# zubair-irshad/NeO-360

Hardware: AMD Instinct MI355X
Metric: rays/sec (128 samples/ray) + PSNR vs ref, 640x480 (higher is better)
Workload: dtype f32 (fp16-MFMA products of hi/lo-split fp32 operands, fp32 accumulate)

## Files before the change

neo-360_amd/csrc/api_tp.hip:

```cpp
#include "tp_frame.h"

#include <algorithm>

using namespace neo_host;

namespace {

double tp_flop_per_point(int input_ch, int nv) {
    const double per_view = input_ch == 3 ? 255424.0 : 260800.0;
    return 2.0 * (nv * per_view + 4416.0);
}

int ensure_projections(neo_ctx* ctx, MlpSlot& sl, const neo::TpScene& sc, bool planes, hipStream_t s, long plane_base[3],
                       bool split_guard = false) {
    const long t_lat = static_cast<long>(sc.nv) * sc.Hf * sc.Wf, t_pl = static_cast<long>(sc.nv) * sc.Hp * sc.Wp;
    for (int j = 0; j < 3; ++j) plane_base[j] = t_lat + j * t_pl;
    const size_t need = neo::tp_proj_bytes(t_lat + (planes ? 3 * t_pl : 0)) + neo::tp_proj_pad_bytes();
    REQUIRE(need <= 4294967295UL, "projected maps too large for 32-bit byte offsets");
    if (need > sl.proj.cap) {
        if (int rc = ctx->touch_shared(s)) return rc;
        if (sl.proj.reserve(need)) return NEO_ERR_NOMEM;
        sl.proj_weights = sl.proj_scene = sl.projpl_weights = sl.projpl_scene = 0;
    }
    if (sl.proj_weights != sl.weights_epoch || sl.proj_scene != ctx->scene_epoch) {
        if (int rc = ctx->touch_shared(s)) return rc;
        neo::launch_tp_preproject(sc.latent, t_lat, sl.wpack.as<float>(), neo::tp_kc_x(sl.input_ch), sl.proj.as<float>(), s);
        if (split_guard) neo::launch_f32_range_check(sl.proj.as<float>(), static_cast<size_t>(t_lat) * 256, 65504.0f, ctx->flags, s);
        sl.proj_weights = sl.weights_epoch;
        sl.proj_scene = ctx->scene_epoch;
    }
    if (planes && (sl.projpl_weights != sl.weights_epoch || sl.projpl_scene != ctx->scene_epoch)) {
        if (int rc = ctx->touch_shared(s)) return rc;
        for (int j = 0; j < 3; ++j)
            neo::launch_tp_preproject(sc.plane[j], t_pl, sl.wpack.as<float>(), neo::tp_kc_x(sl.input_ch),
                                      sl.proj.as<float>() + plane_base[j] * 256, s, 256, 128, 64);
        if (split_guard)
            neo::launch_f32_range_check(sl.proj.as<float>() + plane_base[0] * 256, static_cast<size_t>(3 * t_pl) * 256, 65504.0f / 3.0f, ctx->flags, s);
        sl.projpl_weights = sl.weights_epoch;
        sl.projpl_scene = ctx->scene_epoch;
    }
    return NEO_OK;
}

int guard_planes_low(neo_ctx* ctx, const neo::TpScene& sc, hipStream_t s) {
    if (ctx->planes_low_checked == ctx->scene_epoch) return NEO_OK;
    if (int rc = ctx->touch_shared(s)) return rc;
    if (int rc = guard_map_low(ctx, MAP_MAX_PLANES, sc.plane, 3, static_cast<size_t>(sc.nv) * sc.Hp * sc.Wp * 128, neo::SPLIT_MAP_LOW,
                               true, s)) return rc;
    ctx->planes_low_checked = ctx->scene_epoch;
    return NEO_OK;
}

int tp_launch(neo_ctx* ctx, MlpSlot& sl, const neo::TpScene& sc, const neo::TpViews& views, const float* rays_o,
              const float* rays_d, const float* viewdirs, const float* tvals, const float* far, int R, int N, int chunk,
              float* out, hipStream_t s, const int* cull_map = nullptr, const int* cull_count = nullptr,
              bool density_only = false) {
    ORDERED(ctx, s);
    const int slot_index = static_cast<int>(&sl - ctx->tp);
    neo::TpScene scp = sc;
    if (cull_map) {
        scp.cull_map = cull_map;
        scp.cull_count = cull_count;
        scp.grid_w = 0;
    }
    if (scp.grid_w > 0) {
        static int epw = -2, eph = -2;
        if (epw == -2) {
            epw = eph = -1;
            if (const char* e = getenv("NEO_TP_PATCH")) (void)sscanf(e, "%d,%d", &epw, &eph);
        }
        scp.grid_pw = epw >= 0 ? epw : (slot_index < 2 ? 1 : 3);
        scp.grid_ph = eph >= 0 ? eph : (slot_index < 2 ? 1 : 3);
        if (scp.grid_w % (1 << scp.grid_pw) != 0) scp.grid_w = 0;
    }
    {
        static const int quad_default[4] = {16, 16, 16, 16};
        static int equad = -2;
        if (equad == -2) {
            const char* e = getenv("NEO_TP_QUAD");
            const int v = e ? atoi(e) : -1;
            equad = v == 1 ? 4 : (v == 0 || v == 4 || v == 8 || v == 16) ? v : -1;
        }
        const int forced = ctx->tp_quad >= 0 ? ctx->tp_quad : equad;
        scp.quad = cull_map ? 0 : forced >= 0 ? forced : quad_default[slot_index];
    }
    long plane_base[3] = {0, 0, 0};
    if (ctx->precision == 1) {
        if (ctx->planes_checked != ctx->scene_epoch) {
            const size_t n = static_cast<size_t>(sc.nv) * sc.Hp * sc.Wp * 128;
            for (int j = 0; j < 3; ++j) neo::launch_f32_range_check(sc.plane[j], n, 65504.0f / 3.0f, ctx->flags, s);
            ctx->planes_checked = ctx->scene_epoch;
        }
        if (ctx->preproject) {
            const bool planes = ctx->preproject == 2 || (ctx->preproject == 3 && slot_index >= 2);
            if (int rc = ensure_projections(ctx, sl, sc, planes, s, plane_base, true)) return rc;
            guard_split_weights(sl, sl.wpack_hp.p, neo::tp_wpack_hp_bytes(sl.input_ch), ctx->flags, s, neo::SPLIT_WEIGHT_LOW_TP, 1u << 6);
            if (!planes)
                if (int rc = guard_planes_low(ctx, sc, s)) return rc;
            neo::TpMlpHDev mh{sl.wpack_hp.p, sl.bias_hp.as<float>(), sl.heads.as<float>(), ctx->flags};
            const bool dens = density_only && !(cull_map && sl.input_ch == 3);
            if (ctx->tp_dirsum->reserve(static_cast<size_t>(R) * 32 * sizeof(float))) return NEO_ERR_NOMEM;
            if (!dens) neo::launch_tp_dirsum(viewdirs, R, views, sc.nv, ctx->tp_dirsum->as<float>(), s);
            ctx->span_kernel_next = planes ? 2 : 1;
            ctx->span_begin(s);
            if (planes)
                neo::launch_tp_mlp_hpp(sl.input_ch, mh, sl.proj.as<float>(), plane_base, scp, views, rays_o, rays_d, viewdirs, tvals, far,
                                       R, N, chunk, ctx->flags, out, ctx->tp_dirsum->as<float>(), s, dens);
            else
                neo::launch_tp_mlp_hp(sl.input_ch, mh, sl.proj.as<float>(), scp, views, rays_o, rays_d, viewdirs, tvals, far, R, N,
                                      chunk, ctx->flags, out, ctx->tp_dirsum->as<float>(), s, dens);
        } else {
            guard_split_weights(sl, sl.wpack_h.p, neo::tp_wpack_h_bytes(sl.input_ch), ctx->flags, s, neo::SPLIT_WEIGHT_LOW_TP);
            if (ctx->latent_checked != ctx->scene_epoch) {
                neo::launch_f32_range_check(sc.latent, static_cast<size_t>(sc.nv) * sc.Hf * sc.Wf * 512, 65504.0f, ctx->flags, s);
                ctx->latent_checked = ctx->scene_epoch;
            }
            if (int rc = guard_planes_low(ctx, sc, s)) return rc;
            if (ctx->latent_low_checked != ctx->scene_epoch) {
                if (int rc = ctx->touch_shared(s)) return rc;
                if (int rc = guard_map_low(ctx, MAP_MAX_LATENT, &sc.latent, 1, static_cast<size_t>(sc.nv) * sc.Hf * sc.Wf * 512,
                                           neo::SPLIT_MAP_LOW, true, s)) return rc;
                ctx->latent_low_checked = ctx->scene_epoch;
            }
            neo::TpMlpHDev mh{sl.wpack_h.p, sl.bias.as<float>(), sl.heads.as<float>(), ctx->flags};
            ctx->span_kernel_next = 3;
            ctx->span_begin(s);
            neo::launch_tp_mlp_h(sl.input_ch, mh, scp, views, rays_o, rays_d, viewdirs, tvals, far, R, N, chunk, ctx->flags, out, s);
        }
    } else {
        neo::TpMlpDev m{sl.wpack.as<float>(), sl.bias.as<float>(), sl.heads.as<float>()};
        const bool planes = ctx->preproject >= 2;
        if (ctx->preproject)
            if (int rc = ensure_projections(ctx, sl, sc, planes, s, plane_base)) return rc;
        const float* pbase = sl.proj.as<float>();
        const neo::TpPlaneProj pp{{pbase + plane_base[0] * 256, pbase + plane_base[1] * 256, pbase + plane_base[2] * 256}};
        if (ctx->preproject) {
            if (ctx->tp_dirsum->reserve(static_cast<size_t>(R) * 32 * sizeof(float))) return NEO_ERR_NOMEM;
            neo::launch_tp_dirsum(viewdirs, R, views, sc.nv, ctx->tp_dirsum->as<float>(), s);
        }
        ctx->span_kernel_next = 4;
        ctx->span_begin(s);
        neo::launch_tp_mlp(sl.input_ch, m, scp, views, rays_o, rays_d, viewdirs, tvals, far, R, N, chunk, ctx->flags, out, s,
                           ctx->preproject ? sl.proj.as<float>() : nullptr, planes ? &pp : nullptr,
                           ctx->preproject ? ctx->tp_dirsum->as<float>() : nullptr);
    }
    ctx->span_end(s, cull_map ? 0.0 : static_cast<double>(R) * N, tp_flop_per_point(sl.input_ch, sc.nv));
    return NEO_OK;
}

constexpr int SKIP_WINDOW_DEFAULT = 4096;

int tp_eval_skipping(neo_ctx* ctx, const TpFrame& f, const TpFrameArgs& a, int level, const float* fg_t, int N, float* fg_out,
                     uint8_t* keep, long long* kept) {
    hipStream_t s = f.s;
    const int win = std::min(ctx->skip_window > 0 ? ctx->skip_window : SKIP_WINDOW_DEFAULT, a.R);
    const size_t cap = static_cast<size_t>(win) * N;
    REQUIRE(cap * 3 <= 2147483647UL, "skip window too large for 32-bit indices");
    if (ctx->ws[12].reserve(neo::occ_rows_bytes(cap)) || (!keep && ctx->ws[13].reserve(cap))) return NEO_ERR_NOMEM;
    neo::OccRows w;
    w.carve(ctx->ws[12].p, cap);
    const uint32_t* bits = ctx->occ_G ? ctx->occ_bits.as<uint32_t>() : nullptr;
    if (kept) HIP_TRY(hipMemsetAsync(kept, 0, sizeof(long long), s));
    neo::launch_occ_iota(w.iota, static_cast<int>(cap), s);
    for (int r0 = 0; r0 < a.R; r0 += win) {
        const int rays = std::min(win, a.R - r0);
        const int P = rays * N;
        const size_t first = static_cast<size_t>(r0) * N;
        uint8_t* keep_win = keep ? keep + first : ctx->ws[13].as<uint8_t>();
        neo::launch_occ_compact(a.rays_o, a.rays_d, a.viewdirs, fg_t + first, r0, rays, a.R, N, a.chunk, bits, ctx->occ_G, keep_win,
                                w, kept, s);
        if (int rc = tp_launch(ctx, ctx->tp[level], f.sc, f.views, w.o, w.d, w.v, w.t, nullptr, P, 1, a.chunk, w.out, s, w.iota, w.count))
            return rc;
        neo::launch_occ_scatter(keep_win, P, w, fg_out + first * 4, s);
    }
    return NEO_OK;
}

struct TpTermState {
    double* carry;
    float* trans;
    int* stop;
    int* cws;
    static size_t bytes(size_t r, int win) { return r * 16 + neo::cull_ws_ints(win) * sizeof(int); }
    void carve(void* base, size_t r) {
        carry = static_cast<double*>(base);
        trans = reinterpret_cast<float*>(carry + r);
        stop = reinterpret_cast<int*>(trans + r);
        cws = stop + r;
    }
};

int tp_eval_terminating(neo_ctx* ctx, const TpFrame& f, const TpFrameArgs& a, int level, const float* fg_t, const float* far, int N,
                        float* fg_out, float eps, int segment, const TpTermState& st, int win, long long* kept) {
    hipStream_t s = f.s;
    const int seg = std::min(segment, N);
    const size_t cap = static_cast<size_t>(win) * seg;
    if (ctx->ws[12].reserve(neo::occ_rows_bytes(cap))) return NEO_ERR_NOMEM;
    neo::OccRows w;
    w.carve(ctx->ws[12].p, cap);
    HIP_TRY(hipMemsetAsync(fg_out, 0, static_cast<size_t>(a.R) * N * 16, s));
    neo::launch_term_init(st.trans, st.stop, a.R, 0, kept, 0, s);
    neo::launch_occ_iota(w.iota, static_cast<int>(cap), s);
    for (int r0 = 0; r0 < a.R; r0 += win) {
        const int rays = std::min(win, a.R - r0);
        for (int b0 = 0; b0 < N; b0 += segment) {
            const int len = std::min(segment, N - b0);
            const int P = rays * len;
            neo::launch_cull_compact(st.trans + r0, st.trans + r0, rays, eps, st.cws, nullptr, s);
            const int* map_w = neo::cull_map_of(st.cws, rays);
            const int* count_w = neo::cull_count_of(st.cws, rays);
            neo::launch_term_emit(a.rays_o, a.rays_d, a.viewdirs, fg_t, map_w, count_w, r0, rays, a.R, N, b0, len, a.chunk, w, kept, s);
            if (int rc = tp_launch(ctx, ctx->tp[level], f.sc, f.views, w.o, w.d, w.v, w.t, nullptr, P, 1, a.chunk, w.out, s, w.iota, w.count))
                return rc;
            neo::launch_term_scatter(w, P, fg_out, s);
            neo::launch_term_advance(fg_out, fg_t, a.rays_d, far, N, b0, b0 + len, segment, eps, map_w, count_w, rays, r0, st.carry,
                                     st.trans, st.stop, s);
        }
    }
    return NEO_OK;
}

bool level0_sigma_only(const neo_tp_level_out* level0) {
    return !level0 || !(level0->rgb || level0->fg_rgb || level0->bg_rgb || level0->depth);
}

}

int neo_tp_eval_region(neo_ctx* ctx, int slot, const neo::TpScene& sc, const neo::TpViews& views, const float* rays_o,
                       const float* rays_d, const float* viewdirs, const float* tvals, const float* far, int R, int N,
                       int chunk, float* out, hipStream_t s) {
    MlpSlot& sl = ctx->tp[slot];
    if (!sl.ready) return fail(NEO_ERR_STATE, "NeRF_TP MLP slot %d has no weights", slot);
    return tp_launch(ctx, sl, sc, views, rays_o, rays_d, viewdirs, tvals, far, R, N, chunk, out, s);
}

namespace neo_host {

int TpFrame::begin(neo_ctx* c, const TpFrameArgs& a, bool outside, bool use_grid, const Own& own) {
    ctx = c;
    s = static_cast<hipStream_t>(a.stream);
    REQUIRE(a.R >= 0 && a.chunk >= 1, "bad ray count / chunk");
    REQUIRE(!own.after_rays, own.after_rays);
    REQUIRE(a.n_coarse >= 3 && a.n_coarse <= 256 && a.n_fine >= 1 && a.n_coarse + 1 + a.n_fine <= 1024, "unsupported sample counts");
    REQUIRE(!own.after_counts, own.after_counts);
    if (a.R == 0 || own.empty) {
        empty = true;
        return NEO_OK;
    }
    REQUIRE(a.rays_o && a.rays_d && a.viewdirs && a.src_poses && own.ptrs, "null pointer");
    REQUIRE(!own.after_ptrs, own.after_ptrs);
    if (!ctx->scene_ready) return fail(NEO_ERR_STATE, "scene features not set (neo_tp_set_scene)");
    REQUIRE(a.NV == ctx->scene.nv, "NV differs from the uploaded scene");
    for (int i = 0; i < (outside ? 4 : 2); ++i)
        if (!ctx->tp[i].ready) return fail(NEO_ERR_STATE, "NeRF_TP MLP slot %d has no weights", i);
    if (outside)
        REQUIRE(ctx->tp[0].input_ch == 3 && ctx->tp[1].input_ch == 3 && ctx->tp[2].input_ch == 4 && ctx->tp[3].input_ch == 4,
                "slots 0,1 must be fg (input_ch 3), slots 2,3 bg (input_ch 4)");
    else
        REQUIRE(ctx->tp[0].input_ch == 3 && ctx->tp[1].input_ch == 3, "slots 0,1 must be fg (input_ch 3)");
    const CallScene cs = call_scene(ctx->scene, a.src_poses, a.NV, a.focal, a.cx, a.cy);
    sc = cs.sc;
    views = cs.views;
    if (use_grid) {
        sc.grid_w = ctx->ray_grid_w;
        sc.grid_first = ctx->ray_grid_first;
    }
    N0 = a.n_coarse + 1;
    N1 = N0 + a.n_fine;
    edges = ctx->get_edges(a.n_coarse, 0.0f, 1.0f, s);
    u = ctx->get_quantiles(a.n_fine, s);
    if (!edges || !u) return fail(NEO_ERR_HIP, "constant table upload failed");
    if (int rc = ctx->order_begin(s, true)) return rc;
    ordered = true;
    return NEO_OK;
}

int tp_render_dense(neo_ctx* ctx, const TpFrameArgs& a, const TpDenseOptions& o) {
    TpFrame::Own own;
    bool want_extras[2];
    for (int l = 0; l < 2; ++l) {
        const neo_tp_extras_out* ex = o.extras[l];
        want_extras[l] = ex && (ex->opacity || ex->disparity || (ex->dist_pct && o.n_u > 0));
        if (!own.after_counts && ex && ex->dist_pct && o.n_u > 0 && !o.u_extras) own.after_counts = "null quantile table";
    }
    if (!(o.n_u >= 0 && o.n_u <= 8)) own.after_counts = "bad quantile count (0 <= n_u <= 8)";
    if (!((o.K_edit == 0 && o.K_dec == 0) || (o.near_inst && o.far_inst))) own.after_ptrs = "null interval pointer";
    else if (!(o.L == 0 || (o.layers && o.layers->key && o.layers->rgb && o.layers->acc && o.layers->depth)))
        own.after_ptrs = "null layer pointer";
    TpFrame f;
    if (int rc = f.begin(ctx, a, true, true, own)) return rc;
    if (f.empty) return NEO_OK;
    hipStream_t s = f.s;
    const int R = a.R, chunk = a.chunk, N0 = f.N0, N1 = f.N1;
    const float *rays_o = a.rays_o, *rays_d = a.rays_d, *viewdirs = a.viewdirs;

    auto* W = ctx->ws;
    const size_t r = static_cast<size_t>(R);
    const bool want_fg_w1 = want_extras[1] || o.decomposed[1] || (o.samples[1] && o.samples[1]->fg_w);
    TpDenseRows rows;
    if (rows.reserve(W, r, N0, N1) || W[9].reserve(r * 16 * 4)) return NEO_ERR_NOMEM;
    if (want_fg_w1 && W[10].reserve(r * N1 * 4)) return NEO_ERR_NOMEM;
    if (want_extras[1] && W[11].reserve(r * N1 * 4)) return NEO_ERR_NOMEM;
    auto [far, fg_t0, bg_s0, fg_out, bg_out, fg_w0, bg_w0, fg_t1, bg_s1] = rows;
    float* fg_w1 = want_fg_w1 ? W[10].as<float>() : nullptr;
    float* bg_w1 = want_extras[1] ? W[11].as<float>() : nullptr;
    float* scratch = W[9].as<float>();
    float* s_fg_rgb = scratch;
    float* s_fg_depth = scratch + r * 3;
    float* s_fg_acc = scratch + r * 4;
    float* s_lambda = scratch + r * 5;
    float* s_bg_rgb = scratch + r * 6;
    float* s_bg_depth = scratch + r * 9;

    neo::launch_sphere(rays_o, rays_d, R, far, nullptr, ctx->flags, s);
    neo::launch_tp_level0(far, f.edges, R, N0, f.near, fg_t0, bg_s0, s);

    const bool sigma0 = o.level0_may_be_sigma_only && level0_sigma_only(o.level[0]);
    const float* fg_t = fg_t0;
    const float* bg_s = bg_s0;
    for (int level = 0; level < 2; ++level) {
        const int N = level == 0 ? N0 : N1;
        const neo_tp_level_out* lo = o.level[level];
        const neo_tp_edit_samples* so = o.samples[level];
        const neo_tp_decomposed_out* dc = o.decomposed[level];
        const bool dens = level == 0 && sigma0;
        if (o.skip) {
            if (int rc = tp_eval_skipping(ctx, f, a, level, fg_t, N, fg_out, o.fg_keep[level], o.kept ? o.kept + level : nullptr)) return rc;
            if (o.fg_rows[level]) HIP_TRY(hipMemcpyAsync(o.fg_rows[level], fg_out, r * N * 16, hipMemcpyDeviceToDevice, s));
        } else if (int rc = tp_launch(ctx, ctx->tp[level], f.sc, f.views, rays_o, rays_d, viewdirs, fg_t, nullptr, R, N, chunk, fg_out, s, nullptr, nullptr, dens)) return rc;
        if (int rc = tp_launch(ctx, ctx->tp[2 + level], f.sc, f.views, rays_o, rays_d, viewdirs, bg_s, far, R, N, chunk, bg_out, s, nullptr, nullptr, dens)) return rc;
        float* fg_rgb = dens ? nullptr : (lo && lo->fg_rgb) ? lo->fg_rgb : s_fg_rgb;
        float* bg_rgb = dens ? nullptr : (lo && lo->bg_rgb) ? lo->bg_rgb : s_bg_rgb;
        float* fg_acc = (lo && lo->fg_acc) ? lo->fg_acc : s_fg_acc;
        float* lam = (lo && lo->bg_lambda) ? lo->bg_lambda : s_lambda;
        float* fg_w = level == 0 ? fg_w0 : fg_w1;
        float* bg_w = level == 0 ? bg_w0 : bg_w1;
        if (o.K_edit > 0) neo::launch_tp_edit(fg_out, fg_t, o.near_inst, o.far_inst, o.K_edit, R, N, *o.edit, s);
        if (o.L > 0)
            neo::launch_composite_layers(fg_out, fg_t, rays_d, far, R, N, o.layers->key, o.layers->rgb, o.layers->acc, o.layers->depth,
                                         o.L, fg_rgb, fg_acc, dens ? nullptr : s_fg_depth, fg_w, lam, so ? so->visibility : nullptr, s);
        else
            neo::launch_composite(1, fg_out, fg_t, N, rays_d, far, R, N, 0, fg_rgb, fg_acc, dens ? nullptr : s_fg_depth, fg_w, lam, s);
        if (dc)
            neo::launch_tp_decompose(fg_out, fg_t, fg_w, o.near_inst, o.far_inst, o.K_dec, R, N, lam, dc->rgb, dc->acc, dc->depth, dc->id, s);
        neo::launch_composite(2, bg_out, bg_s, N, nullptr, nullptr, R, N, 0, bg_rgb, nullptr, dens ? nullptr : s_bg_depth, bg_w,
                              nullptr, s);
        if (lo && (lo->rgb || lo->depth))
            neo::launch_tp_merge(fg_rgb, s_fg_depth, lam, bg_rgb, s_bg_depth, R, lo->rgb, lo->depth, s);
        if (want_extras[level]) {
            const neo_tp_extras_out* ex = o.extras[level];
            if (neo::launch_tp_extras(fg_t, fg_w, far, bg_s, bg_w, lam, rays_o, rays_d, R, N, o.u_extras, o.n_u, ex->opacity,
                                      ex->disparity, ex->dist_pct, s))
                return fail(NEO_ERR_INVALID, "unsupported sample or quantile count");
        }
        if (so) {
            const size_t row = r * N * sizeof(float);
            if (so->fg_t) HIP_TRY(hipMemcpyAsync(so->fg_t, fg_t, row, hipMemcpyDeviceToDevice, s));
            if (so->bg_s) HIP_TRY(hipMemcpyAsync(so->bg_s, bg_s, row, hipMemcpyDeviceToDevice, s));
            if (so->fg_w) HIP_TRY(hipMemcpyAsync(so->fg_w, fg_w, row, hipMemcpyDeviceToDevice, s));
        }
        if (level == 0) {
            if (neo::launch_resample(fg_t0, N0, fg_w0, f.u, 0, R, N0, a.n_fine, 0, fg_t1, s) ||
                neo::launch_resample(bg_s0, N0, bg_w0, f.u, 0, R, N0, a.n_fine, 1, bg_s1, s))
                return fail(NEO_ERR_INVALID, "unsupported sample counts");
            fg_t = fg_t1;
            bg_s = bg_s1;
        }
    }
    return check_launch();
}

int tp_march_compact(const TpFrame& f, const TpFrameArgs& a, const TpCompactRows& c, const int* map, const int* count, int white) {
    neo_ctx* ctx = f.ctx;
    hipStream_t s = f.s;
    const int R = a.R, N0 = f.N0, N1 = f.N1;
    if (int rc = tp_launch(ctx, ctx->tp[0], f.sc, f.views, a.rays_o, a.rays_d, a.viewdirs, c.t0, nullptr, R, N0, a.chunk, c.out, s, map, count)) return rc;
    neo::launch_composite(1, c.out, c.t0, N0, c.rays_d, c.far, R, N0, white, c.rgb[0], c.acc[0], c.depth[0], c.w0, nullptr, s, count);
    if (neo::launch_resample(c.t0, N0, c.w0, f.u, 0, R, N0, a.n_fine, 0, c.t1, s, count)) return fail(NEO_ERR_INVALID, "unsupported sample counts");
    if (int rc = tp_launch(ctx, ctx->tp[1], f.sc, f.views, a.rays_o, a.rays_d, a.viewdirs, c.t1, nullptr, R, N1, a.chunk, c.out, s, map, count)) return rc;
    neo::launch_composite(1, c.out, c.t1, N1, c.rays_d, c.far, R, N1, white, c.rgb[1], c.acc[1], c.depth[1], nullptr, nullptr, s, count);
    return NEO_OK;
}

}

extern "C" {

int neo_tp_upload_mlp(neo_ctx* ctx, int slot, int input_ch, const float* const* weights,
                      const float* const* biases, void* stream) {
    ENTER(ctx);
    ORDERED(ctx, static_cast<hipStream_t>(stream));
    REQUIRE(slot >= 0 && slot < 4, "slot must be 0..3 (fg_coarse, fg_fine, bg_coarse, bg_fine)");
    REQUIRE(input_ch == 3 || input_ch == 4, "input_ch must be 3 (fg) or 4 (bg)");
    REQUIRE(weights && biases, "null pointer table");
    for (int i = 0; i < 9; ++i) REQUIRE(weights[i] && biases[i], "null layer pointer");
    MlpSlot& sl = ctx->tp[slot];
    if (sl.wpack.reserve(neo::tp_wpack_floats(input_ch) * sizeof(float))) return NEO_ERR_NOMEM;
    if (sl.bias.reserve(neo::tp_bias_floats() * sizeof(float))) return NEO_ERR_NOMEM;
    if (sl.heads.reserve(neo::tp_heads_floats() * sizeof(float))) return NEO_ERR_NOMEM;
    if (sl.wpack_h.reserve(neo::tp_wpack_h_bytes(input_ch))) return NEO_ERR_NOMEM;
// ... 363 lines not shown
```

neo-360_amd/csrc/mlp_tp_hpp.hip:

```cpp
#include <hip/hip_fp16.h>

#include <algorithm>
#include <cstdlib>
#include <type_traits>

#include "tp_hp_layout.h"

#ifndef NEO_TPP_WPS
#define NEO_TPP_WPS 2
#endif
#ifndef NEO_TPP_RING
#define NEO_TPP_RING 3
#endif
#ifndef NEO_TPP_XD
#define NEO_TPP_XD 1
#endif
#ifndef NEO_TPP_LD
#define NEO_TPP_LD 4
#endif
#ifndef NEO_TPP_TD
#define NEO_TPP_TD 6
#endif
#define TPP_SYNC() __syncthreads()
#ifndef NEO_TP_TRACE
#define NEO_TP_TRACE 0
#endif
#if NEO_TP_TRACE
__device__ unsigned long long g_tpp_trace[16];
#define TPP_MARK(k) do { const unsigned long long now_ = __builtin_amdgcn_s_memtime(); tr_[k] += now_ - tlast_; tlast_ = now_; } while (0)
#else
#define TPP_MARK(k) do { } while (0)
#endif

namespace neo {

namespace {

using namespace hp;
constexpr int RING = NEO_TPP_RING;

constexpr int PP_OFF_DESC = tp::OFF_DIR + TM * 32;
constexpr int DESC_BLOCK = TM * 4, DESC_W = 5 * DESC_BLOCK;
constexpr int PP_OFF_LIST = PP_OFF_DESC + 2 * DESC_W;
constexpr int LIST_MAX = 18;
constexpr int PP_OFF_CAM = PP_OFF_LIST + 4 * LIST_MAX * 4;
constexpr int PP_OFF_PE = PP_OFF_CAM + TM * 4;
constexpr int PP_OFF_FEAT = PP_OFF_PE + TM * 4;
constexpr int PP_OFF_VDIR = PP_OFF_FEAT + TM * 4;
constexpr int PP_OFF_DENSW = PP_OFF_VDIR + TM * 4;
constexpr int PP_OFF_BIAS = PP_OFF_DENSW + 128;
constexpr int PP_OFF_XPE0 = PP_OFF_BIAS + 768 + 336;
constexpr int PP_LDS_WORDS = PP_OFF_XPE0 + TM * 64;
static_assert(PP_LDS_WORDS * 4 <= 81920, "two workgroups per CU");

struct TpPlaneBase { int texels[3]; };

template <int PE_C, bool CULL = false, bool DENS = false>
__global__ __launch_bounds__(256, NEO_TPP_WPS) void k_tp_mlp_hpp(TpMlpHDev m, const float* __restrict__ proj, TpPlaneBase plb,
                                                               TpScene sc, TpViews views, const float* __restrict__ rays_o,
                                                               const float* __restrict__ rays_d,
                                                               const float* __restrict__ viewdirs,
                                                               const float* __restrict__ tvals,
                                                               const float* __restrict__ far_arr, int R, int N, int chunk,
                                                               uint32_t* __restrict__ flags, float4* __restrict__ out,
                                                               const float* __restrict__ dirsum) {
    extern __shared__ __attribute__((aligned(16))) float smem[];
    _Float16* hbase = reinterpret_cast<_Float16*>(smem + tp::OFF_ACT);
    const HT act{hbase, hbase + TM * 128};
    auto fbuf = [&](int b) { return smem + tp::OFF_ACT + b * (TM * 64); };
    _Float16* xb0 = reinterpret_cast<_Float16*>(smem + PP_OFF_XPE0);
    const HT xpe0{xb0, xb0 + TM * 64};
    _Float16* dbase = reinterpret_cast<_Float16*>(smem + tp::OFF_DIR);
    const HT dsm{dbase, dbase + TM * 32};
    const HT xpe1 = dsm;
    tp::Scratch S;
    S.loc_off = reinterpret_cast<int*>(smem + PP_OFF_DESC);
    S.pl_off = S.loc_off + DESC_BLOCK;
    S.loc_w = smem + PP_OFF_DESC + DESC_W;
    S.pl_w = S.loc_w + DESC_BLOCK;
    S.cam_enc = smem + PP_OFF_CAM;
    S.pe_world = smem + PP_OFF_PE;
    S.feat_world = smem + PP_OFF_FEAT;
    S.vdir_world = smem + PP_OFF_VDIR;
    [[maybe_unused]] int* loc_off = S.loc_off;
    float* loc_w = S.loc_w;
    [[maybe_unused]] int* pl_off = S.pl_off;

    LaneCtx L;
    L.init();
    int tid = threadIdx.x;
    const long P = tp::launch_points<CULL>(sc, R, N);
    const long tile0 = tp::xcd_tile<CULL>(blockIdx.x, (P + TM - 1) / TM) * TM;
    if (tile0 >= P) return;
    const h8* wp = reinterpret_cast<const h8*>(m.wpack);
    constexpr int KSX = ks_x(PE_C);
    constexpr int KSP = pe_ksteps(PE_C);
    constexpr int NPE = PE_C == 3 ? 1 : 2;

#if NEO_TP_TRACE
    unsigned long long tr_[8] = {0, 0, 0, 0, 0, 0, 0, 0}, tlast_ = __builtin_amdgcn_s_memtime();
#endif
    tp::point_setup<PE_C>(S, tid, tile0, P, N, R, chunk, rays_o, rays_d, viewdirs, tvals, far_arr, flags, false, sc.grid_w, sc.grid_first, sc.grid_pw, sc.grid_ph, CULL ? sc.cull_map : nullptr, CULL ? 0 : sc.quad);
    float* dens_w = smem + PP_OFF_DENSW;
    if (tid < 128) dens_w[tid] = m.heads[HD_DW + tid];
    if (tid < DESC_BLOCK) {
        S.loc_off[4 * DESC_BLOCK + tid] = 0;
        S.loc_w[4 * DESC_BLOCK + tid] = 0.0f;
    }
    float* lbias_w = smem + PP_OFF_BIAS;
    for (int i = tid; i < 768; i += 256) lbias_w[i] = m.bias[i];
    for (int i = tid; i < HD_RB + 3; i += 256) lbias_w[768 + i] = m.heads[i];
    const float* lbias = lbias_w;
    const float* lheads = lbias_w + 768;
    TPP_SYNC();

    f32x16 hsum[2];
#pragma unroll
    for (int r = 0; r < 16; ++r) { hsum[0][r] = 0.f; hsum[1][r] = 0.f; }
    const int vnt = L.wv & 1, vmt = L.wv >> 1;

    TPP_MARK(0);
#pragma unroll 1
    for (int v = 0; v < sc.nv; ++v) {
        asm volatile("" : "+v"(tid));
        L.lane = tid & 63;
        L.half = L.lane >> 5;
        L.l31 = L.lane & 31;
        L.key = L.lane & 15;
        const float* rot = views.rot[v];
        const float* trn = views.trans[v];
        tp::view_descriptors<PROJ_TEXEL_BYTES, false, PROJ_TEXEL_BYTES>(S, L, sc, rot, trn, v, [](int, int, float) {},
                                                                        L.wv == 0 ? 0 : plb.texels[L.wv == 0 ? 0 : L.wv - 1]);
        {
            const int row = tid & 63, q = tid >> 6;
            const float ex = S.pe_world[row * 4], ey = S.pe_world[row * 4 + 1], ez = S.pe_world[row * 4 + 2];
            f32x4 xv;
            xv[0] = (rot[0] * ex + rot[1] * ey + rot[2] * ez) + trn[0];
            xv[1] = (rot[3] * ex + rot[4] * ey + rot[5] * ez) + trn[1];
            xv[2] = (rot[6] * ex + rot[7] * ey + rot[8] * ez) + trn[2];
            xv[3] = S.pe_world[row * 4 + 3];
            auto pe_chunk = [&](auto ldh, const HT& buf, int pstage, int hf) __attribute__((always_inline)) {
                constexpr int LDH = decltype(ldh)::value;
                const int chs = hf * 4 + q;
                const int ch = pstage * 8 + chs;
                float f[8];
                h8 vh, vl;
                if (ch * 4 < 10 * PE_C) {
#pragma unroll
                    for (int jj = 0; jj < 4; ++jj) {
                        if (PE_C == 3 && jj >= 2 && ch == 7) {
                            f[2 * jj] = jj == 2 ? xv[0] : xv[2];
                            f[2 * jj + 1] = jj == 2 ? xv[1] : 0.0f;
                            range_see(L, f[2 * jj]); range_see(L, f[2 * jj + 1]);
                            continue;
                        }
                        float x;
                        int oct;
                        if constexpr (PE_C == 4) {
                            x = xv[jj];
                            oct = ch;
                        } else {
                            const int p = ch * 4 + jj;
                            oct = p / 3;
                            const int a = p - 3 * oct;
                            x = a == 0 ? xv[0] : a == 1 ? xv[1] : xv[2];
                        }
                        sincos_pair(ldexpf(x, oct), f[2 * jj], f[2 * jj + 1]);
                    }
                } else {
#pragma unroll
                    for (int e = 0; e < 8; ++e) f[e] = 0.0f;
                    if (ch * 4 == 10 * PE_C) {
                        range_see(L, xv[0]); range_see(L, xv[1]); range_see(L, xv[2]); range_see(L, xv[3]);
                        f[0] = xv[0]; f[1] = xv[1]; f[2] = xv[2]; f[3] = xv[3];
                    }
                }
#pragma unroll
                for (int e = 0; e < 8; e += 2) {
                    h2 h, l;
                    split2(f[e], f[e + 1], h, l);
                    vh[e] = h[0]; vh[e + 1] = h[1];
                    vl[e] = l[0]; vl[e + 1] = l[1];
                }
                const int o = chunk_off<LDH>(row, chs);
                *reinterpret_cast<h8*>(buf.hi + o) = vh;
                *reinterpret_cast<h8*>(buf.lo + o) = vl;
            };
            pe_chunk(std::integral_constant<int, 64>(), xpe0, 0, 0);
            pe_chunk(std::integral_constant<int, 64>(), xpe0, 0, 1);
            if constexpr (NPE == 2) pe_chunk(std::integral_constant<int, 32>(), xpe1, 1, 0);
        }
        TPP_SYNC();
        TPP_MARK(1);

        f32x16 accx[2][2];
        bias_tile(accx[0][0], lbias + B_0, L.wv, L);
        bias_tile(accx[1][0], lbias + B_3, L.wv, L);
        accx[0][1] = accx[0][0];
        accx[1][1] = accx[1][0];
        {
            const int col4 = tid & 15, rg = tid >> 4;
            const uint32_t lane_b = 16u * col4;
            f32x4 taps[RING][4];
            f32x4 wsum;
            int4 d_off[RING];
            [[maybe_unused]] f32x4 d_w[2];
            f32x4 d_w3[RING];
            constexpr int XD = NEO_TPP_XD, XS = XD + 1;
            h8 wh[XS][2], wl[XS][2];
            const char* wxb = reinterpret_cast<const char*>(wp + hoff_x());
            uint32_t wx_off[2];
            wx_off[0] = (uint32_t)((L.wv * KSX + 8) * 2 * 64 + L.lane) * 16u;
            wx_off[1] = (uint32_t)(((4 + L.wv) * KSX + 8) * 2 * 64 + L.lane) * 16u;
            auto load_wk = [&](auto kc) __attribute__((always_inline)) {
                constexpr int kp = decltype(kc)::value;
                if constexpr (kp < KSP) {
#pragma unroll
                    for (int nt = 0; nt < 2; ++nt) {
                        wh[kp % XS][nt] = *reinterpret_cast<const h8*>(wxb + (wx_off[nt] + 2048u * kp));
                        wl[kp % XS][nt] = *reinterpret_cast<const h8*>(wxb + (wx_off[nt] + 2048u * kp + 1024u));
                    }
                }
            };
            auto mma_k = [&](auto kc) __attribute__((always_inline)) {
                constexpr int kp = decltype(kc)::value;
                h8 bh[2], bl[2];
#pragma unroll
                for (int mt = 0; mt < 2; ++mt) {
                    if constexpr (kp < 4) {
                        const int o = chunk_off<64>(mt * 32 + L.l31, (kp << 1) + L.half);
                        bh[mt] = *reinterpret_cast<const h8*>(xpe0.hi + o);
                        bl[mt] = *reinterpret_cast<const h8*>(xpe0.lo + o);
                    } else {
                        const int o = chunk_off<32>(mt * 32 + L.l31, ((kp - 4) << 1) + L.half);
                        bh[mt] = *reinterpret_cast<const h8*>(xpe1.hi + o);
                        bl[mt] = *reinterpret_cast<const h8*>(xpe1.lo + o);
                    }
                }
#pragma unroll
                for (int nt = 0; nt < 2; ++nt)
#pragma unroll
                    for (int mt = 0; mt < 2; ++mt) {
                        accx[nt][mt] = NEO_MFMA_H_LH(wl[kp % XS][nt], bh[mt], accx[nt][mt]);
                        accx[nt][mt] = NEO_MFMA_H_HL(wh[kp % XS][nt], bl[mt], accx[nt][mt]);
                        accx[nt][mt] = NEO_MFMA_H(wh[kp % XS][nt], bh[mt], accx[nt][mt]);
                    }
                load_wk(std::integral_constant<int, kp + XD>());
            };
            auto consume_chunk = [&](auto cc) __attribute__((always_inline)) {
                constexpr int c = decltype(cc)::value;
                const float* buf = fbuf(c & 1);
#pragma unroll
                for (int mt = 0; mt < 2; ++mt)
#pragma unroll
                    for (int gg = 0; gg < 2; ++gg) {
                        const int row = mt * 32 + L.l31;
                        const int piece = L.wv * 4 + gg * 2 + L.half;
                        const f32x4 val = *reinterpret_cast<const f32x4*>(buf + row * 64 + ((piece ^ (row & 15)) << 2));
                        constexpr int g0 = 2 * (c & 1);
#pragma unroll
                        for (int e = 0; e < 4; ++e) accx[c >> 1][mt][4 * (g0 + gg) + e] += val[e];
                    }
            };
            static_assert(RING == 3 && LIST_MAX % RING == 0, "the work-list pipeline is written for a ring of three");
            int n_p;
            bool any_w;
            const int4* list;
            {
                int4* mylist = reinterpret_cast<int4*>(smem + PP_OFF_LIST) + L.wv * LIST_MAX;
                unsigned am = 0;
#pragma unroll
                for (int mp = 0; mp < 4; ++mp) {
                    const f32x4 w = *reinterpret_cast<const f32x4*>(loc_w + (mp * TM + L.lane) * 4);
                    const unsigned long long z = __ballot(w[0] != 0.0f || w[1] != 0.0f || w[2] != 0.0f || w[3] != 0.0f);
#pragma unroll
                    for (int q = 0; q < 4; ++q) am |= (((z >> (16 * q)) & 0xFFFFull) != 0ull ? 1u : 0u) << (4 * q + mp);
                }
                any_w = am != 0u;
#pragma unroll
                for (int q = 0; q < 4; ++q)
                    if (((am >> (4 * q)) & 0xFu) == 0u) am |= 1u << (4 * q);
                const int n = __builtin_popcount(am);
                n_p = ((n + RING - 1) / RING) * RING;
                {
                    const int b = L.lane;
                    const bool real = b < 16 && ((am >> b) & 1u);
                    const bool pad = b - 32 >= n && b - 32 < n_p;
                    if (real || pad) {
                        int4 rec;
                        int at = b - 32;
                        if (real) {
                            const int q = b >> 2, mp = b & 3;
                            const unsigned grp = (am >> (4 * q)) & 0xFu;
                            rec.x = (mp * TM + 16 * q) * 16;
                            rec.y = 16 * q;
                            rec.z = (grp & ((1u << mp) - 1u)) == 0u ? 0 : 0x3f800000;
                            rec.w = (grp >> (mp + 1)) == 0u ? 1 : 0;
                            at = __builtin_popcount(am & ((1u << b) - 1u));
                        } else {
                            rec.x = 4 * DESC_BLOCK * 4;
                            rec.y = 0;
                            rec.z = 0x3f800000;
                            rec.w = 0;
                        }
                        mylist[at] = rec;
                    }
                }
                list = mylist;
            }
            const char* dbase = reinterpret_cast<const char*>(S.loc_off) + rg * 16;
            float* fstore = fbuf(0) + rg * 64 + ((col4 ^ rg) << 2);
            auto wrap = [&](int idx) __attribute__((always_inline)) { return idx >= n_p ? idx - n_p : idx; };
            int rx[RING];
            int4 fin[RING];
#pragma unroll
            for (int e = 0; e < 4; ++e) wsum[e] = 0.0f;
            static_for<0, XD>([&](auto kc) { load_wk(kc); });
            if (any_w) {
                const int r0 = list[0].x, r1 = list[1].x, r2 = list[2].x;
                fin[0] = list[0];
                rx[0] = list[3].x; rx[1] = r1; rx[2] = r2;
                const int4 o0 = *reinterpret_cast<const int4*>(dbase + r0);
                const int4 o1 = *reinterpret_cast<const int4*>(dbase + r1);
                d_off[2] = *reinterpret_cast<const int4*>(dbase + r2);
                d_w3[0] = *reinterpret_cast<const f32x4*>(dbase + r0 + DESC_W * 4);
                taps[0][0] = tp::load_tap(proj, (uint32_t)o0.x + lane_b); taps[0][1] = tp::load_tap(proj, (uint32_t)o0.y + lane_b);
                taps[0][2] = tp::load_tap(proj, (uint32_t)o0.z + lane_b); taps[0][3] = tp::load_tap(proj, (uint32_t)o0.w + lane_b);
                taps[1][0] = tp::load_tap(proj, (uint32_t)o1.x + lane_b); taps[1][1] = tp::load_tap(proj, (uint32_t)o1.y + lane_b);
                taps[1][2] = tp::load_tap(proj, (uint32_t)o1.z + lane_b); taps[1][3] = tp::load_tap(proj, (uint32_t)o1.w + lane_b);
            }
            TPP_MARK(2);
            auto step = [&](auto cc, auto jc, int k) __attribute__((always_inline)) {
                constexpr int c = decltype(cc)::value, j = decltype(jc)::value;
                constexpr int j1 = (j + 1) % RING, j2 = (j + 2) % RING;
                const int e = k + j;
                d_w3[j1] = *reinterpret_cast<const f32x4*>(dbase + rx[j1] + DESC_W * 4);
                rx[j1] = list[wrap(e + 4)].x;
                fin[j1] = list[wrap(e + 1)];
                d_off[j] = *reinterpret_cast<const int4*>(dbase + rx[j]);
                {
                    const float* base = proj + 64 * (e + 2 >= n_p ? c + 1 : c);
                    const int4 off = d_off[j2];
                    taps[j2][0] = tp::load_tap(base, (uint32_t)off.x + lane_b);
                    taps[j2][1] = tp::load_tap(base, (uint32_t)off.y + lane_b);
                    taps[j2][2] = tp::load_tap(base, (uint32_t)off.z + lane_b);
                    taps[j2][3] = tp::load_tap(base, (uint32_t)off.w + lane_b);
                }
                const f32x4 val = blend4(taps[j], d_w3[j]);
                const float keep = __int_as_float(fin[j].z);
#pragma unroll
                for (int t = 0; t < 4; ++t) wsum[t] = __builtin_fmaf(wsum[t], keep, val[t]);
                if (fin[j].w) *reinterpret_cast<f32x4*>(fstore + (c & 1) * (TM * 64) + fin[j].y * 64) = wsum;
                __builtin_amdgcn_sched_barrier(0);
            };
            if (!any_w) n_p = 0;
            static_for<0, 4>([&](auto cc) {
                constexpr int c = decltype(cc)::value;
                static_for<0, KSP>([&](auto kc) {
                    constexpr int kp = decltype(kc)::value;
                    if constexpr ((KSP == 4 ? kp : (kp < 2 ? 0 : kp < 3 ? 1 : kp < 5 ? 2 : 3)) == c) mma_k(kc);
                });
#pragma unroll 1
                for (int k = 0; k < n_p; k += RING) static_for<0, RING>([&](auto jc) { step(cc, jc, k); });
                TPP_SYNC();
                if (any_w)
                consume_chunk(cc);
            });
        }
        TPP_SYNC();
        TPP_MARK(3);
        {
            constexpr int LD = NEO_TPP_LD, LS = LD + 1;
            h8 lwh[LS], lwl[LS];
            const char* lwb = reinterpret_cast<const char*>(wp);
            const uint32_t lw_off = (uint32_t)(L.wv * 8 * 128 + L.lane) * 16u;
            auto load_l = [&](auto gc) __attribute__((always_inline)) {
                constexpr int g = decltype(gc)::value;
                if constexpr (g < 24) {
                    constexpr int layer = g / 8, ks = g % 8;
                    constexpr uint32_t base = (uint32_t)(layer == 0 ? hoff_1(PE_C) : layer == 1 ? hoff_2(PE_C) : hoff_3a(PE_C)) * 16u;
                    lwh[g % LS] = *reinterpret_cast<const h8*>(lwb + (base + lw_off + 2048u * ks));
                    lwl[g % LS] = *reinterpret_cast<const h8*>(lwb + (base + lw_off + 2048u * ks + 1024u));
                }
            };
            static_for<0, LD>([&](auto gc) { load_l(gc); });
            f32x16 acc[2];
            store_tile_h<true>(accx[0][0], act, L.wv, 0, L);
            store_tile_h<true>(accx[0][1], act, L.wv, 1, L);
            TPP_SYNC();
            static_for<0, 24>([&](auto gc) {
                constexpr int g = decltype(gc)::value;
                constexpr int layer = g / 8, ks = g % 8;
                if constexpr (ks == 0) {
                    if constexpr (layer < 2) {
                        bias_tile(acc[0], lbias + (layer == 0 ? B_1 : B_2), L.wv, L);
                        acc[1] = acc[0];
                    } else {
                        acc[0] = accx[1][0];
                        acc[1] = accx[1][1];
                    }
                }
                load_l(std::integral_constant<int, g + LD>());
                h8 bh[2], bl[2];
#pragma unroll
                for (int mt = 0; mt < 2; ++mt) {
                    const int o = chunk_off<128>(mt * 32 + L.l31, (ks << 1) + L.half);
                    bh[mt] = *reinterpret_cast<const h8*>(act.hi + o);
                    bl[mt] = *reinterpret_cast<const h8*>(act.lo + o);
                }
#pragma unroll
                for (int mt = 0; mt < 2; ++mt) {
                    acc[mt] = NEO_MFMA_H_LH(lwl[g % LS], bh[mt], acc[mt]);
                    acc[mt] = NEO_MFMA_H_HL(lwh[g % LS], bl[mt], acc[mt]);
                    acc[mt] = NEO_MFMA_H(lwh[g % LS], bh[mt], acc[mt]);
                }
                if constexpr (ks == 7) {
                    if constexpr (layer < 2) {
                        TPP_SYNC();
                        store_tile_h<true>(acc[0], act, L.wv, 0, L);
                        store_tile_h<true>(acc[1], act, L.wv, 1, L);
                        TPP_SYNC();
                    } else {
#pragma unroll
                        for (int r = 0; r < 16; ++r) {
                            hsum[0][r] += relu1(acc[0][r]);
                            hsum[1][r] += relu1(acc[1][r]);
                        }
                    }
                }
                __builtin_amdgcn_sched_barrier(0);
            });
        }
        TPP_SYNC();
        TPP_MARK(4);
    }

    const float inv_nv = 1.0f / (float)sc.nv;
#pragma unroll
    for (int r = 0; r < 16; ++r) { hsum[0][r] = hsum[0][r] * inv_nv; hsum[1][r] = hsum[1][r] * inv_nv; }
    store_tile_h<false>(hsum[0], act, L.wv, 0, L);
    store_tile_h<false>(hsum[1], act, L.wv, 1, L);
    if constexpr (!DENS) {
        const int p = tid >> 2, f0 = (tid & 3) << 3;
        const int dray = __float_as_int(S.vdir_world[p * 4 + 3]);
        const f32x4 s0 = *reinterpret_cast<const f32x4*>(dirsum + (long)dray * 32 + f0);
        const f32x4 s1 = *reinterpret_cast<const f32x4*>(dirsum + (long)dray * 32 + f0 + 4);
        h8 vh, vl;
#pragma unroll
        for (int j = 0; j < 8; j += 2) {
            const float a = (j < 4 ? s0[j] : s1[j - 4]) * inv_nv, b = (j < 4 ? s0[j + 1] : s1[j - 3]) * inv_nv;
            h2 h, l;
            split2(a, b, h, l);
            vh[j] = h[0]; vh[j + 1] = h[1];
            vl[j] = l[0]; vl[j + 1] = l[1];
        }
        const int o = chunk_off<32>(p, tid & 3);
        *reinterpret_cast<h8*>(dsm.hi + o) = vh;
        *reinterpret_cast<h8*>(dsm.lo + o) = vl;
    }
    TPP_SYNC();
    float raw_sigma;
    {
        float sg = density_partial(act, dens_w, L);
        sg += __shfl_xor(sg, 1, 64);
        sg += __shfl_xor(sg, 2, 64);
        raw_sigma = sg + lheads[HD_DB];
    }
    if constexpr (!DENS) {
        const char* twb = reinterpret_cast<const char*>(wp);
        constexpr int TD = NEO_TPP_TD, TS = TD + 1;
        h8 twh[TS], twl[TS];
        auto load_t = [&](auto gc) __attribute__((always_inline)) {
            constexpr int g = decltype(gc)::value;
            if constexpr (g < 14) {
                constexpr bool v0 = g < 10;
                constexpr int ks = v0 ? g : g - 10;
                constexpr int KS = v0 ? 10 : 4;
                constexpr uint32_t base = (uint32_t)(v0 ? hoff_v0(PE_C) : hoff_v1(PE_C)) * 16u;
                const uint32_t off = base + (uint32_t)((vnt * KS + ks) * 128 + L.lane) * 16u;
                twh[g % TS] = *reinterpret_cast<const h8*>(twb + off);
                twl[g % TS] = *reinterpret_cast<const h8*>(twb + off + 1024u);
            }
        };
        static_for<0, TD>([&](auto gc) { load_t(gc); });
        f32x16 y;
        static_for<0, 14>([&](auto gc) {
            constexpr int g = decltype(gc)::value;
            load_t(std::integral_constant<int, g + TD>());
            constexpr bool v0 = g < 10;
            constexpr int ks = v0 ? g : g - 10;
            if constexpr (ks == 0) bias_tile(y, lbias + (v0 ? B_V0 : B_V1), vnt, L);
            h8 bh, bl;
            if constexpr (v0 && ks >= 8) {
                const int o = chunk_off<32>(vmt * 32 + L.l31, ((ks - 8) << 1) + L.half);
                bh = *reinterpret_cast<const h8*>(dsm.hi + o);
                bl = *reinterpret_cast<const h8*>(dsm.lo + o);
            } else {
                const int o = chunk_off<128>(vmt * 32 + L.l31, (ks << 1) + L.half);
                bh = *reinterpret_cast<const h8*>(act.hi + o);
                bl = *reinterpret_cast<const h8*>(act.lo + o);
            }
            y = NEO_MFMA_H_LH(twl[g % TS], bh, y);
            y = NEO_MFMA_H_HL(twh[g % TS], bl, y);
            y = NEO_MFMA_H(twh[g % TS], bh, y);
            if constexpr (g == 9) {
                TPP_SYNC();
                store_tile_h<true>(y, act, vnt, vmt, L);
                TPP_SYNC();
            }
            if constexpr (g == 13) {
                TPP_SYNC();
                store_tile_h<true>(y, act, vnt, vmt, L);
            }
            __builtin_amdgcn_sched_barrier(0);
        });
        TPP_SYNC();
    }
    {
        const int pt = L.wv * 16 + (L.lane >> 2), part = L.lane & 3;
        [[maybe_unused]] float r = 0.f, g = 0.f, b = 0.f;
        if constexpr (!DENS) {
            const float* wr = lheads + HD_RW;
#pragma unroll
            for (int c = 0; c < 2; ++c) {
                const int chunk_i = part * 2 + ((c + part) & 1);
                const int o = chunk_off<128>(pt, chunk_i);
                const h8 vh = *reinterpret_cast<const h8*>(act.hi + o);
                const h8 vl = *reinterpret_cast<const h8*>(act.lo + o);
#pragma unroll
                for (int e = 0; e < 8; ++e) {
                    const float h = (float)vh[e] + (float)vl[e];
                    r += h * wr[chunk_i * 8 + e];
                    g += h * wr[64 + chunk_i * 8 + e];
                    b += h * wr[128 + chunk_i * 8 + e];
                }
            }
            r += __shfl_xor(r, 1, 64); r += __shfl_xor(r, 2, 64);
            g += __shfl_xor(g, 1, 64); g += __shfl_xor(g, 2, 64);
            b += __shfl_xor(b, 1, 64); b += __shfl_xor(b, 2, 64);
        }
        range_commit(L, m.flags);
        const long gv = tile0 + pt;
        const long gi = tp::launch_point(gv, N, R, CULL ? 0 : sc.quad, sc.grid_w, sc.grid_first, sc.grid_pw, sc.grid_ph);
        if (part == 0 && gv < P) {
            if constexpr (DENS)
                out[gi] = make_float4(0.0f, 0.0f, 0.0f, density_act(raw_sigma));
            else
                out[gi] = make_float4(colour_act(r + lheads[HD_RB]), colour_act(g + lheads[HD_RB + 1]),
                                      colour_act(b + lheads[HD_RB + 2]), density_act(raw_sigma));
        }
    }
#if NEO_TP_TRACE
    TPP_MARK(5);
    if (threadIdx.x == 0) {
#pragma unroll
        for (int k = 0; k < 6; ++k) atomicAdd(&g_tpp_trace[k], tr_[k]);
        atomicAdd(&g_tpp_trace[7], 1ull);
    }
#endif
}

}

#if NEO_TP_TRACE
extern "C" void neo_debug_tpp_trace(unsigned long long* host16, int reset) {
    (void)hipDeviceSynchronize();
    (void)hipMemcpyFromSymbol(host16, HIP_SYMBOL(g_tpp_trace), sizeof(unsigned long long) * 16);
    if (reset) {
        unsigned long long z[16] = {0};
        (void)hipMemcpyToSymbol(HIP_SYMBOL(g_tpp_trace), z, sizeof(z));
    }
}
#endif

void launch_tp_mlp_hpp(int input_ch, const TpMlpHDev& m, const float* proj_all, const long plane_base_texels[3],
                       const TpScene& sc, const TpViews& views, const float* rays_o, const float* rays_d, const float* viewdirs,
                       const float* tvals, const float* far, int R, int N, int chunk, uint32_t* flags, float* out,
                       const float* dirsum, hipStream_t s, bool density_only) {
    const long P = (long)R * N;
    if (P <= 0) return;
    const float* proj = proj_all;
    const TpPlaneBase pp{{(int)plane_base_texels[0], (int)plane_base_texels[1], (int)plane_base_texels[2]}};
    const size_t lds = (size_t)PP_LDS_WORDS * sizeof(float);
    static bool attr_set[64] = {};
    int dev = 0;
    (void)hipGetDevice(&dev);
    if (dev < 0 || dev >= 64 || !attr_set[dev]) {
        (void)hipFuncSetAttribute(reinterpret_cast<const void*>(k_tp_mlp_hpp<3>), hipFuncAttributeMaxDynamicSharedMemorySize, (int)lds);
        (void)hipFuncSetAttribute(reinterpret_cast<const void*>(k_tp_mlp_hpp<4>), hipFuncAttributeMaxDynamicSharedMemorySize, (int)lds);
        (void)hipFuncSetAttribute(reinterpret_cast<const void*>(k_tp_mlp_hpp<4, true>), hipFuncAttributeMaxDynamicSharedMemorySize, (int)lds);
        (void)hipFuncSetAttribute(reinterpret_cast<const void*>(k_tp_mlp_hpp<3, true>), hipFuncAttributeMaxDynamicSharedMemorySize, (int)lds);
        (void)hipFuncSetAttribute(reinterpret_cast<const void*>(k_tp_mlp_hpp<3, false, true>), hipFuncAttributeMaxDynamicSharedMemorySize, (int)lds);
        (void)hipFuncSetAttribute(reinterpret_cast<const void*>(k_tp_mlp_hpp<4, false, true>), hipFuncAttributeMaxDynamicSharedMemorySize, (int)lds);
        (void)hipFuncSetAttribute(reinterpret_cast<const void*>(k_tp_mlp_hpp<4, true, true>), hipFuncAttributeMaxDynamicSharedMemorySize, (int)lds);
        if (dev >= 0 && dev < 64) attr_set[dev] = true;
    }
    const long tiles = tp::xcd_grid((P + TM - 1) / TM);
    const bool dens = density_only && !(sc.cull_map && input_ch == 3);
    if (dens) {
    } else if (!sc.cull_map && input_ch == 3)
        hipLaunchKernelGGL(k_tp_mlp_hpp<3>, dim3((unsigned)tiles), dim3(256), lds, s, m, proj, pp, sc, views, rays_o, rays_d,
                           viewdirs, tvals, far, R, N, chunk, flags, reinterpret_cast<float4*>(out), dirsum);
    else if (sc.cull_map && input_ch != 3)
        hipLaunchKernelGGL((k_tp_mlp_hpp<4, true>), dim3((unsigned)tiles), dim3(256), lds, s, m, proj, pp, sc, views, rays_o, rays_d,
                           viewdirs, tvals, far, R, N, chunk, flags, reinterpret_cast<float4*>(out), dirsum);
    else if (!sc.cull_map)
        hipLaunchKernelGGL(k_tp_mlp_hpp<4>, dim3((unsigned)tiles), dim3(256), lds, s, m, proj, pp, sc, views, rays_o, rays_d,
                           viewdirs, tvals, far, R, N, chunk, flags, reinterpret_cast<float4*>(out), dirsum);
    else
        hipLaunchKernelGGL((k_tp_mlp_hpp<3, true>), dim3((unsigned)tiles), dim3(256), lds, s, m, proj, pp, sc, views, rays_o, rays_d,
                           viewdirs, tvals, far, R, N, chunk, flags, reinterpret_cast<float4*>(out), dirsum);
    if (!dens) return;
    if (!sc.cull_map && input_ch == 3)
        hipLaunchKernelGGL((k_tp_mlp_hpp<3, false, true>), dim3((unsigned)tiles), dim3(256), lds, s, m, proj, pp, sc, views, rays_o, rays_d,
                           viewdirs, tvals, far, R, N, chunk, flags, reinterpret_cast<float4*>(out), dirsum);
    else if (!sc.cull_map)
        hipLaunchKernelGGL((k_tp_mlp_hpp<4, false, true>), dim3((unsigned)tiles), dim3(256), lds, s, m, proj, pp, sc, views, rays_o, rays_d,
                           viewdirs, tvals, far, R, N, chunk, flags, reinterpret_cast<float4*>(out), dirsum);
    else
        hipLaunchKernelGGL((k_tp_mlp_hpp<4, true, true>), dim3((unsigned)tiles), dim3(256), lds, s, m, proj, pp, sc, views, rays_o, rays_d,
                           viewdirs, tvals, far, R, N, chunk, flags, reinterpret_cast<float4*>(out), dirsum);
}

}
```

Baseline: 527,400.

## Add static fully-unrolled tap pipeline for dense inside-sphere plane-projection launch

Adds a STATIC template variant of the plane-projected TP MLP kernel for the non-culled, 3-channel case. It replaces the runtime work-list pipeline with a compile-time unrolled ring of tap loads, using 4 or 3 taps per group depending on a wave ballot of latent weights. The goal is to remove work-list construction and branching so loads can overlap MMA. It becomes the default for that case and can be switched off with an environment variable. It also introduces a per-slot planes_default table and keeps the low-plane guard on slots below 2 in preproject mode 3, at the cost of more template instantiations and code size.

```diff
diff --git a/neo-360_amd/csrc/api_tp.hip b/neo-360_amd/csrc/api_tp.hip
--- a/neo-360_amd/csrc/api_tp.hip
+++ b/neo-360_amd/csrc/api_tp.hip
@@ -84,6 +84,7 @@
         const int forced = ctx->tp_quad >= 0 ? ctx->tp_quad : equad;
         scp.quad = cull_map ? 0 : forced >= 0 ? forced : quad_default[slot_index];
     }
+    static const bool planes_default[4] = {false, false, true, true};
     long plane_base[3] = {0, 0, 0};
     if (ctx->precision == 1) {
         if (ctx->planes_checked != ctx->scene_epoch) {
@@ -92,10 +93,10 @@
             ctx->planes_checked = ctx->scene_epoch;
         }
         if (ctx->preproject) {
-            const bool planes = ctx->preproject == 2 || (ctx->preproject == 3 && slot_index >= 2);
+            const bool planes = ctx->preproject == 2 || (ctx->preproject == 3 && planes_default[slot_index]);
             if (int rc = ensure_projections(ctx, sl, sc, planes, s, plane_base, true)) return rc;
             guard_split_weights(sl, sl.wpack_hp.p, neo::tp_wpack_hp_bytes(sl.input_ch), ctx->flags, s, neo::SPLIT_WEIGHT_LOW_TP, 1u << 6);
-            if (!planes)
+            if (!planes || (ctx->preproject == 3 && slot_index < 2))
                 if (int rc = guard_planes_low(ctx, sc, s)) return rc;
             neo::TpMlpHDev mh{sl.wpack_hp.p, sl.bias_hp.as<float>(), sl.heads.as<float>(), ctx->flags};
             const bool dens = density_only && !(cull_map && sl.input_ch == 3);
diff --git a/neo-360_amd/csrc/mlp_tp_hpp.hip b/neo-360_amd/csrc/mlp_tp_hpp.hip
--- a/neo-360_amd/csrc/mlp_tp_hpp.hip
+++ b/neo-360_amd/csrc/mlp_tp_hpp.hip
@@ -55,7 +55,7 @@
 
 struct TpPlaneBase { int texels[3]; };
 
-template <int PE_C, bool CULL = false, bool DENS = false>
+template <int PE_C, bool CULL = false, bool DENS = false, bool STATIC = false>
 __global__ __launch_bounds__(256, NEO_TPP_WPS) void k_tp_mlp_hpp(TpMlpHDev m, const float* __restrict__ proj, TpPlaneBase plb,
                                                                TpScene sc, TpViews views, const float* __restrict__ rays_o,
                                                                const float* __restrict__ rays_d,
@@ -64,6 +64,7 @@
                                                                const float* __restrict__ far_arr, int R, int N, int chunk,
                                                                uint32_t* __restrict__ flags, float4* __restrict__ out,
                                                                const float* __restrict__ dirsum) {
+    static_assert(!STATIC || (PE_C == 3 && !CULL), "the static form is the dense inside-sphere launch's");
     extern __shared__ __attribute__((aligned(16))) float smem[];
     _Float16* hbase = reinterpret_cast<_Float16*>(smem + tp::OFF_ACT);
     const HT act{hbase, hbase + TM * 128};
@@ -205,7 +206,7 @@
             f32x4 wsum;
             int4 d_off[RING];
             [[maybe_unused]] f32x4 d_w[2];
-            f32x4 d_w3[RING];
+            [[maybe_unused]] f32x4 d_w3[RING];
             constexpr int XD = NEO_TPP_XD, XS = XD + 1;
             h8 wh[XS][2], wl[XS][2];
             const char* wxb = reinterpret_cast<const char*>(wp + hoff_x());
@@ -262,6 +263,74 @@
                         for (int e = 0; e < 4; ++e) accx[c >> 1][mt][4 * (g0 + gg) + e] += val[e];
                     }
             };
+            if constexpr (STATIC) {
+            static_assert(RING == 3, "a G = 3 chunk is padded to 13 items for a ring of three");
+            bool any_latent;
+            {
+                const f32x4 w0 = *reinterpret_cast<const f32x4*>(loc_w + L.lane * 4);
+                any_latent = __ballot(w0[0] != 0.0f || w0[1] != 0.0f || w0[2] != 0.0f || w0[3] != 0.0f) != 0ull;
+            }
+            auto fetch_off = [&](auto gc, auto ic) __attribute__((always_inline)) {
+                constexpr int G = decltype(gc)::value, NL = G == 4 ? 16 : 13, i = decltype(ic)::value, l = i % NL;
+                if constexpr (i < 4 * NL && l < 4 * G)
+                    d_off[l & 1] = *reinterpret_cast<const int4*>(loc_off + ((l % G + (4 - G)) * TM + rg + 16 * (l / G)) * 4);
+            };
+            auto fetch_w = [&](auto gc, auto ic) __attribute__((always_inline)) {
+                constexpr int G = decltype(gc)::value, NL = G == 4 ? 16 : 13, i = decltype(ic)::value, l = i % NL;
+                if constexpr (i < 4 * NL && l < 4 * G)
+                    d_w[l & 1] = *reinterpret_cast<const f32x4*>(loc_w + ((l % G + (4 - G)) * TM + rg + 16 * (l / G)) * 4);
+            };
+            auto issue = [&](auto gc, auto ic) __attribute__((always_inline)) {
+                constexpr int G = decltype(gc)::value, NL = G == 4 ? 16 : 13, i = decltype(ic)::value, l = i % NL;
+                if constexpr (i < 4 * NL && l < 4 * G) {
+                    constexpr int c = i / NL;
+                    const int4 off = d_off[l & 1];
+                    taps[i % RING][0] = tp::load_tap(proj, (uint32_t)off.x + lane_b + 256u * c);
+                    taps[i % RING][1] = tp::load_tap(proj, (uint32_t)off.y + lane_b + 256u * c);
+                    taps[i % RING][2] = tp::load_tap(proj, (uint32_t)off.z + lane_b + 256u * c);
+                    taps[i % RING][3] = tp::load_tap(proj, (uint32_t)off.w + lane_b + 256u * c);
+                }
+            };
+            auto finish = [&](auto gc, auto ic) __attribute__((always_inline)) {
+                constexpr int G = decltype(gc)::value, NL = G == 4 ? 16 : 13, i = decltype(ic)::value, l = i % NL;
+                if constexpr (l < 4 * G) {
+                    constexpr int k = l % G, c = i / NL, q = l / G;
+                    const f32x4 val = blend4(taps[i % RING], d_w[l & 1]);
+                    if constexpr (k == 0) wsum = val; else wsum = wsum + val;
+                    if constexpr (k == G - 1) {
+                        const int row = rg + 16 * q;
+                        *reinterpret_cast<f32x4*>(fbuf(c & 1) + row * 64 + ((col4 ^ (row & 15)) << 2)) = wsum;
+                    }
+                }
+            };
+            auto prologue = [&](auto gc) __attribute__((always_inline)) {
+                static_for<0, RING - 1>([&](auto ic) { fetch_off(gc, ic); issue(gc, ic); });
+                fetch_off(gc, std::integral_constant<int, RING - 1>());
+                fetch_w(gc, std::integral_constant<int, 0>());
+            };
+            auto chunk_items = [&](auto gc, auto cc) __attribute__((always_inline)) {
+                constexpr int G = decltype(gc)::value, NL = G == 4 ? 16 : 13, c = decltype(cc)::value;
+                static_for<NL * c, NL * (c + 1)>([&](auto ic) {
+                    constexpr int i = decltype(ic)::value;
+                    fetch_off(gc, std::integral_constant<int, i + RING>());
+                    fetch_w(gc, std::integral_constant<int, i + 1>());
+                    issue(gc, std::integral_constant<int, i + RING - 1>());
+                    finish(gc, ic);
+                    __builtin_amdgcn_sched_barrier(0);
+                });
+            };
+            static_for<0, XD>([&](auto kc) { load_wk(kc); });
+            if (any_latent) prologue(std::integral_constant<int, 4>());
+            else prologue(std::integral_constant<int, 3>());
+            TPP_MARK(2);
+            static_for<0, 4>([&](auto cc) {
+                mma_k(cc);
+                if (any_latent) chunk_items(std::integral_constant<int, 4>(), cc);
+                else chunk_items(std::integral_constant<int, 3>(), cc);
+                TPP_SYNC();
+                consume_chunk(cc);
+            });
+            } else {
             static_assert(RING == 3 && LIST_MAX % RING == 0, "the work-list pipeline is written for a ring of three");
             int n_p;
             bool any_w;
@@ -366,6 +435,7 @@
                 if (any_w)
                 consume_chunk(cc);
             });
+            }
         }
         TPP_SYNC();
         TPP_MARK(3);
@@ -593,11 +663,19 @@
         (void)hipFuncSetAttribute(reinterpret_cast<const void*>(k_tp_mlp_hpp<3, false, true>), hipFuncAttributeMaxDynamicSharedMemorySize, (int)lds);
         (void)hipFuncSetAttribute(reinterpret_cast<const void*>(k_tp_mlp_hpp<4, false, true>), hipFuncAttributeMaxDynamicSharedMemorySize, (int)lds);
         (void)hipFuncSetAttribute(reinterpret_cast<const void*>(k_tp_mlp_hpp<4, true, true>), hipFuncAttributeMaxDynamicSharedMemorySize, (int)lds);
+        (void)hipFuncSetAttribute(reinterpret_cast<const void*>(k_tp_mlp_hpp<3, false, false, true>), hipFuncAttributeMaxDynamicSharedMemorySize, (int)lds);
+        (void)hipFuncSetAttribute(reinterpret_cast<const void*>(k_tp_mlp_hpp<3, false, true, true>), hipFuncAttributeMaxDynamicSharedMemorySize, (int)lds);
         if (dev >= 0 && dev < 64) attr_set[dev] = true;
     }
     const long tiles = tp::xcd_grid((P + TM - 1) / TM);
     const bool dens = density_only && !(sc.cull_map && input_ch == 3);
-    if (dens) {
+    static int worklist_env = -1;
+    if (worklist_env < 0) {
+        const char* e = getenv("NEO_TP_PLANES_WORKLIST");
+        worklist_env = e && atoi(e) != 0 ? 1 : 0;
+    }
+    const bool stat = !sc.cull_map && input_ch == 3 && !worklist_env;
+    if (dens || stat) {
     } else if (!sc.cull_map && input_ch == 3)
         hipLaunchKernelGGL(k_tp_mlp_hpp<3>, dim3((unsigned)tiles), dim3(256), lds, s, m, proj, pp, sc, views, rays_o, rays_d,
                            viewdirs, tvals, far, R, N, chunk, flags, reinterpret_cast<float4*>(out), dirsum);
@@ -610,6 +688,15 @@
     else
         hipLaunchKernelGGL((k_tp_mlp_hpp<3, true>), dim3((unsigned)tiles), dim3(256), lds, s, m, proj, pp, sc, views, rays_o, rays_d,
                            viewdirs, tvals, far, R, N, chunk, flags, reinterpret_cast<float4*>(out), dirsum);
+    if (stat) {
+        if (dens)
+            hipLaunchKernelGGL((k_tp_mlp_hpp<3, false, true, true>), dim3((unsigned)tiles), dim3(256), lds, s, m, proj, pp, sc, views, rays_o, rays_d,
+                               viewdirs, tvals, far, R, N, chunk, flags, reinterpret_cast<float4*>(out), dirsum);
+        else
+            hipLaunchKernelGGL((k_tp_mlp_hpp<3, false, false, true>), dim3((unsigned)tiles), dim3(256), lds, s, m, proj, pp, sc, views, rays_o, rays_d,
+                               viewdirs, tvals, far, R, N, chunk, flags, reinterpret_cast<float4*>(out), dirsum);
+        return;
+    }
     if (!dens) return;
     if (!sc.cull_map && input_ch == 3)
         hipLaunchKernelGGL((k_tp_mlp_hpp<3, false, true>), dim3((unsigned)tiles), dim3(256), lds, s, m, proj, pp, sc, views, rays_o, rays_d,
```

After: 527,400. About the same (-0.0%).
